# johannah/drqv2

Hardware: AMD Instinct MI355X
Metric: agent updates/sec (batch=256, 9x84x84 obs) (higher is better)
Workload: dtype f32; 1 GPU; cheetah_run batch_size=256/GPU (256 global) 9x84x84 u8 obs, A=6, feature_dim=50, hidden_dim=1024, fp32, use_tb=True; parallelism=dp1, global_batch=256

## Files before the change

drqv2_amd/_lib.py:

```python
import ctypes as C
import os

HERE = os.path.dirname(os.path.abspath(__file__))
LIB_PATH = os.path.join(HERE, "libdrqv2_hip.so")

c_float_p = C.c_void_p
c_u8_p = C.c_void_p
stream_t = C.c_void_p


class DrqStep(C.Structure):
    _fields_ = [
        ("B", C.c_int), ("global_B", C.c_int), ("C", C.c_int), ("A", C.c_int), ("F", C.c_int), ("H", C.c_int),
        ("obs", c_u8_p), ("next_obs", c_u8_p),
        ("action", c_float_p), ("reward", c_float_p), ("discount", c_float_p),
        ("shift_obs", c_float_p), ("shift_next", c_float_p),
        ("noise_critic", c_float_p), ("noise_actor", c_float_p),
        ("base_grid", c_float_p),
        ("params", c_float_p), ("grads", c_float_p), ("adam_m", c_float_p), ("adam_v", c_float_p),
        ("ws", c_float_p), ("ws_bytes", C.c_size_t),
        ("sums", c_float_p),
        ("lr", C.c_double), ("tau", C.c_double),
        ("std", C.c_float), ("clip", C.c_float),
        ("step_critic", C.c_long), ("step_enc", C.c_long), ("step_actor", C.c_long),
# ... 6 lines not shown
        ("timing_n", C.c_int),
        ("obs_index", C.c_void_p), ("next_obs_index", C.c_void_p),
        ("flags", C.c_int),
    ]


I, L, F, D, P, SZ = C.c_int, C.c_long, C.c_float, C.c_double, C.c_void_p, C.c_size_t

PROTOTYPES = {
    "drq_abi_version": (I, []),
    "drq_aug_fwd": (I, [P, P, P, P, I, I, I, I, I, P]),
    "drq_aug_fwd_f32": (I, [P, P, P, P, I, I, I, I, P]),
    "drq_conv1_aug_fwd": (I, [P, P, P, P, P, P, P, P, P, I, I, P]),
    "drq_conv1_aug_fwd_bf16": (I, [P, P, P, P, P, P, P, P, P, I, I, P]),
    "drq_conv1_aug_fwd_bf16_nhwc": (I, [P, P, P, P, P, P, P, P, P, I, I, P]),
    "drq_conv1_aug_fwd_indexed": (I, [P, P, P, P, P, P, P, P, P, P, P, I, I, P]),
    "drq_conv3x3_fwd": (I, [P, P, P, P, I, I, I, I, I, L, L, L, L, P]),
    "drq_conv3x3_dgrad": (I, [P, P, P, P, I, I, L, L, L, L, P]),
    "drq_conv3x3_fwd_wino": (I, [P, P, P, P, I, I, I, L, L, L, L, P]),
    "drq_conv3x3_dgrad_wino": (I, [P, P, P, P, I, I, L, L, L, L, P]),
    "drq_conv3x3_wgrad_wino": (I, [P, P, P, P, I, I, L, L, L, L, P, SZ, P]),
    "drq_conv3x3_wgrad": (I, [P, P, P, P, I, I, I, I, L, L, L, L, P, SZ, P]),
    "drq_conv3x3_wgrad_ws_bytes": (SZ, []),
    "drq_conv3x3_fwd_bf16": (I, [P, P, P, P, I, I, I, L, L, L, L, P]),
    "drq_conv3x3_dgrad_bf16": (I, [P, P, P, P, I, I, L, L, L, L, P]),
    "drq_conv3x3_wgrad_bf16": (I, [P, P, P, P, I, I, L, L, L, L, P, SZ, P]),
    "drq_conv3x3_fwd_bf16_nhwc": (I, [P, P, P, P, I, I, I, I, I, P]),
    "drq_conv3x3_dgrad_bf16_nhwc": (I, [P, P, P, P, I, I, I, I, L, L, L, L, P]),
    "drq_conv3x3_wgrad_bf16_nhwc": (I, [P, P, P, P, I, I, I, L, L, L, L, P, SZ, P]),
    "drq_gemm_f32": (I, [P, L, I, P, L, I, P, L, I, I, I, I, L, L, L, P, L, I, P, I, L, I, I, I, P, SZ, P]),
    "drq_gemm_batched_f32": (I, [I, P, L, I, P, L, I, P, L, I, I, I, P, I, P, I, P, I, I, I, P, SZ, P]),
    "drq_gemm_batched_bf16": (I, [I, P, L, I, P, L, I, P, L, I, I, I, P, I, P, I, P, I, I, P, SZ, P]),
    "drq_gemm_batched_partial": (I, [I, P, L, I, P, L, I, P, L, I, I, I, P, P, SZ, C.POINTER(I), P]),
    "drq_mlp_fwd": (I, [I, P, L, P, L, P, L, I, I, I, P, I, P, P, C.POINTER(I), P]),
    "drq_mlp_dgrad": (I, [I, P, L, P, L, P, L, I, I, I, P, I, P]),
    "drq_mlp_wgrad_dgrad": (I, [I, P, L, P, L, P, P, P, L, P, L, P, I, I, I, I, P]),
    "drq_ln_l1_fwd": (I, [I, P, P, P, P, P, P, P, P, P, P, P, P, P, P, P, P, P, I, I, I, L, P]),
    "drq_policy_out_l1_fwd": (I, [P, P, P, P, I, I, I, I, I, F, F, I, P, P, P, L, P, P, P, L, I, P, P, P, P]),
    "drq_qout_fwd": (I, [I, P, P, P, P, I, I, P]),
    "drq_qout_bwd": (I, [I, P, P, P, P, P, P, I, I, P]),
    "drq_ln_tanh_fwd_multi": (I, [I, P, I, P, P, P, P, P, P, I, I, P]),
    "drq_ln_tanh_fwd": (I, [P, I, P, P, P, I, P, P, I, I, P]),
    "drq_ln_tanh_fwd2": (I, [P, P, I, P, P, P, P, P, I, P, I, P, P, P, P, I, I, P]),
    "drq_ln_tanh_bwd": (I, [P, I, P, I, P, I, P, P, P, P, P, P, P, I, I, P]),
    "drq_colsum": (I, [P, L, L, P, L, I, I, I, P]),
    "drq_trunc_normal_sample": (I, [P, P, F, F, I, P, P, L, I, I, P]),
    "drq_copy_cols": (I, [P, I, P, L, I, I, P]),
    "drq_td_mse": (I, [P, P, P, P, P, P, P, P, P, I, F, P]),
    "drq_td_mse_w": (I, [P, P, P, P, P, P, P, P, P, P, P, I, F, P]),
    "drq_actor_loss": (I, [P, P, P, L, P, F, P, P, P, I, I, F, P]),
    "drq_actor_dmu": (I, [P, P, L, I, P, P, I, I, P]),
    "drq_actor_loss_bc": (I, [P, P, P, L, P, L, P, F, F, P, P, P, I, I, F, P]),
    "drq_qout_bwd_actor_bc": (I, [P, P, P, L, P, L, P, F, F, I, F, P, P, P, P, I, I, P]),
    "drq_actor_dmu_bc": (I, [P, P, L, I, P, P, L, P, L, F, P, I, I, P]),
    "drq_policy_out_bwd_bc": (I, [P, P, L, I, P, P, L, P, L, F, P, P, P, P, P, I, I, I, P, I, P]),
    "drq_adam_flat": (I, [P, P, P, P, L, D, L, F, P, D, P]),
    "drq_ema_flat": (I, [P, P, L, D, P]),
    "drq_sum_slices": (I, [P, L, I, P, L, P]),
    "drq_adam_reduce_flat": (I, [P, P, L, I, P, P, L, D, L, F, P]),
    "drq_fill": (I, [P, L, F, P]),
    "drq_u8_normalize": (I, [P, P, L, P]),
    "drq_nstep_gather": (I, [P, P, P, P, P, I, I, L, I, F, P, P, P, P, P, P]),
    "drq_tanh": (I, [P, P, L, P]),
    "drq_per_fill": (I, [P, L, L, L, I, P]),
    "drq_per_sample": (I, [P, L, P, I, I, L, D, P, P, P]),
    "drq_per_update": (I, [P, L, P, P, I, D, D, P]),
# ... 75 lines not shown
```

drqv2_amd/csrc/gemm2.hip:

```cpp
#include "common.h"
#include "internal.h"

namespace {

constexpr int MAXB2 = 8;

struct G2Args {
  const float* A[MAXB2];
  const float* B[MAXB2];
  float* C[MAXB2];
  const float* bias[MAXB2];
  const float* aux[MAXB2];
  float* rowsum[MAXB2];
  long lda, ldb, ldc;
  int ldaux;
  int M, N, K;
  int relu;
  unsigned a_bytes, b_bytes;
};

__device__ __forceinline__ int rowmap2(int r, int half) { return (r & 3) + 8 * (r >> 2) + 4 * half; }

template <bool KC>
__device__ __forceinline__ void load_step(float (&v)[16], __amdgpu_buffer_rsrc_t rs, unsigned voff, unsigned soff,
                                          unsigned ldbytes) {
  if constexpr (KC) {
#pragma unroll
    for (int q = 0; q < 4; ++q) {
      const f32x4 t = __builtin_bit_cast(
          f32x4, __builtin_amdgcn_raw_buffer_load_b128(rs, voff, soff + q * 32, 0));
      const float t0 = t[0], t1 = t[1], t2 = t[2], t3 = t[3];
      v[q * 4 + 0] = t0; v[q * 4 + 1] = t1; v[q * 4 + 2] = t2; v[q * 4 + 3] = t3;
    }
  } else {
// ... 375 lines not shown
        lsoff = (unsigned)tt * 128u + (unsigned)(st * 32) * ldb4;
        lld = ldb4;
      }
#pragma unroll
      for (int e = 0; e < 16; e += 2) {
        b[(s + D) % NS][e] = __uint_as_float(
            __builtin_amdgcn_raw_buffer_load_b32(brs, bvoff, lsoff + (8 * (e >> 2) + (e & 3)) * lld, 0));
        b[(s + D) % NS][e + 1] = __uint_as_float(
            __builtin_amdgcn_raw_buffer_load_b32(brs, bvoff, lsoff + (8 * ((e + 1) >> 2) + ((e + 1) & 3)) * lld, 0));
        __builtin_amdgcn_sched_barrier(0);
        acc0 = __builtin_amdgcn_mfma_f32_32x32x2f32(a[s][e], b[s % NS][e], acc0, 0, 0, 0);
        acc1 = __builtin_amdgcn_mfma_f32_32x32x2f32(a[s][e + 1], b[s % NS][e + 1], acc1, 0, 0, 0);
        __builtin_amdgcn_sched_barrier(0);
      }
    }
    const int n = t * 32 + col;
#pragma unroll
    for (int r = 0; r < 16; ++r) {
      const int row = mt * 32 + rowmap2(r, half);
      if (row < g.M) c[(long)row * g.ldc + n] = acc0[r] + acc1[r];
    }
  }
  if (g.rowsum && grp == 0) {
    float rs = 0.f;
#pragma unroll
    for (int s = 0; s < KSTEPS; ++s)
#pragma unroll
      for (int e = 0; e < 16; ++e) rs += a[s][e];
    rs += __shfl_xor(rs, 32);
    if (half == 0 && m < g.M) g.rowsum[m] = rs;
  }
}

}

int drq_trunk_wgrad_ln(const float* A, long lda, const float* B, long ldb, float* C, long ldc, int M, int N, int K,
                       float* rowsum, const float* ln_dln, const float* ln_xhat, float* ln_dgamma, float* ln_dbeta,
                       int ln_rows, int ln_F, hipStream_t st) {
  if (M < 1 || M > 128 || N < 4096 || N % 32 || (K != 128 && K != 256 && K != 512)) return DRQ_EARG;
  if (ln_rows > 0 && (!ln_dln || !ln_xhat || !ln_dgamma || !ln_dbeta || ln_F < 1 || ln_F > 256)) return DRQ_EARG;
  const size_t ab = (size_t)K * lda * 4, bb = (size_t)K * ldb * 4;
  if (ab >= (1ull << 31) || bb >= (1ull << 31)) return DRQ_EARG;
  TWArgs g{A, B, C, rowsum, lda, ldb, ldc, M, N, K, (unsigned)ab, (unsigned)bb,
           ln_dln, ln_xhat, ln_dgamma, ln_dbeta, ln_rows > 0 ? ln_rows : 0, ln_F};
  const int blocks = drq_num_cus() + (ln_rows > 0 ? 1 : 0);
  if (K == 512) hipLaunchKernelGGL((trunk_wgrad_kernel<16>), dim3(blocks), dim3(256), 0, st, g);
  else if (K == 256) hipLaunchKernelGGL((trunk_wgrad_kernel<8>), dim3(blocks), dim3(256), 0, st, g);
  else hipLaunchKernelGGL((trunk_wgrad_kernel<4>), dim3(blocks), dim3(256), 0, st, g);
  DRQ_LAUNCH_CHECK();
  return DRQ_OK;
}

int drq_trunk_wgrad(const float* A, long lda, const float* B, long ldb, float* C, long ldc, int M, int N, int K,
                    float* rowsum, hipStream_t st) {
  return drq_trunk_wgrad_ln(A, lda, B, ldb, C, ldc, M, N, K, rowsum, nullptr, nullptr, nullptr, nullptr, 0, 0, st);
}

int drq_trunk_fwd_partial(int nbatch, const float* const* A, long lda, const float* const* B, long ldb, int M, int N,
                          int K, float* ws, size_t ws_bytes, int* splitk_out, hipStream_t st) {
  if (nbatch <= 0 || nbatch > MAXB2 || M % 32 || M < 32 || N < 1 || N > 128 || K % 32 || K < 4096) return DRQ_EARG;
  if (lda % 4 || ldb % 4 || !ws || ((uintptr_t)ws & 15)) return DRQ_EARG;
  const size_t ab = (size_t)M * lda * 4, bb = (size_t)N * ldb * 4;
  if (ab >= (1ull << 31) || bb >= (1ull << 31)) return DRQ_EARG;
  TrunkArgs g{};
  for (int b = 0; b < nbatch; ++b) {
    if (((uintptr_t)A[b] & 15) || ((uintptr_t)B[b] & 15)) return DRQ_EARG;
    g.A[b] = A[b]; g.B[b] = B[b];
  }
  g.part = ws; g.lda = lda; g.ldb = ldb; g.M = M; g.N = N; g.K = K;
  g.a_bytes = (unsigned)ab; g.b_bytes = (unsigned)bb;
  const int steps = K / 32, cus = drq_num_cus();
  const bool wide = N > 64;
// ... 38 lines not shown
  if (a_kc && !b_kc) return launch2<true, false>(g, nbatch, st);
  return launch2<false, false>(g, nbatch, st);
}

int drq_gemm2_wgrad_dgrad(int nbatch, const float* const* dy, long lddy, const float* const* x, long ldx,
                          float* const* dw, float* const* db, const float* const* w, long ldw, float* const* dx,
                          long lddx, const float* const* mask, int ldmask, int Brows, int Nout, int Kin, hipStream_t st) {
  if (nbatch <= 0 || nbatch > MAXB2 || Brows % 32 || Nout % 32 || Kin % 32 || Brows < 64 || Nout < 64 || Kin < 32)
    return DRQ_EARG;
  if (lddy % 4) return DRQ_EARG;
  G2Args gw{}, gd{};
  for (int b = 0; b < nbatch; ++b) {
    if (!dy[b] || !x[b] || !dw[b] || !w[b] || !dx[b] || ((uintptr_t)dy[b] & 15)) return DRQ_EARG;
    gw.A[b] = dy[b]; gw.B[b] = x[b]; gw.C[b] = dw[b]; gw.rowsum[b] = db ? db[b] : nullptr;
    gd.A[b] = dy[b]; gd.B[b] = w[b]; gd.C[b] = dx[b]; gd.aux[b] = mask ? mask[b] : nullptr;
  }
  gw.lda = lddy; gw.ldb = ldx; gw.ldc = Kin; gw.M = Nout; gw.N = Kin; gw.K = Brows;
  gd.lda = lddy; gd.ldb = ldw; gd.ldc = lddx; gd.ldaux = ldmask; gd.M = Brows; gd.N = Kin; gd.K = Nout;
  const size_t dyb = (size_t)Brows * lddy * 4, xb = (size_t)Brows * ldx * 4, wb = (size_t)Nout * ldw * 4;
  if (dyb >= (1ull << 31) || xb >= (1ull << 31) || wb >= (1ull << 31)) return DRQ_EARG;
  gw.a_bytes = (unsigned)dyb; gw.b_bytes = (unsigned)xb;
  gd.a_bytes = (unsigned)dyb; gd.b_bytes = (unsigned)wb;
  const bool sw = gemm2_split(gw, nbatch), sd = gemm2_split(gd, nbatch);
  const int tw = (gw.M / 32) * (gw.N / 32), td = (gd.M / 32) * (gd.N / 32);
  const int nxw = sw ? tw : (tw + 3) / 4, nxd = sd ? td : (td + 3) / 4;
  const dim3 grid(nxw + nxd, 1, nbatch);
  if (sw && sd) hipLaunchKernelGGL((gemm2_pair_kernel<4, 4>), grid, dim3(256), 0, st, gw, gd, nxw);
  else if (sw) hipLaunchKernelGGL((gemm2_pair_kernel<4, 1>), grid, dim3(256), 0, st, gw, gd, nxw);
  else if (sd) hipLaunchKernelGGL((gemm2_pair_kernel<1, 4>), grid, dim3(256), 0, st, gw, gd, nxw);
  else hipLaunchKernelGGL((gemm2_pair_kernel<1, 1>), grid, dim3(256), 0, st, gw, gd, nxw);
  DRQ_LAUNCH_CHECK();
  return DRQ_OK;
}
```

drqv2_amd/csrc/internal.h:

```cpp
#pragma once
#include "common.h"

int drq_ln_tanh_fwd_multi_ex(int n, const float* const* z, int ldz, const float* const* gamma,
                             const float* const* beta, float* const* out, const int* ldo, float* const* xhat,
                             float* const* rstd, int rows, int F, const float* const* tail, const int* tail_ld,
                             int tail_n, hipStream_t st);
int drq_ln_tanh_fwd_multi_part(int n, const float* const* z, int ldz, const float* const* gamma,
                               const float* const* beta, float* const* out, const int* ldo, float* const* xhat,
                               float* const* rstd, int rows, int F, const float* const* tail, const int* tail_ld,
                               int tail_n, const float* part, const float* const* bias, int splitk, hipStream_t st);
int drq_ln_tanh_bwd_part(const float* dh0, int ld0, const float* dh1, int ld1, const float* h, int ldh,
                         const float* xhat, const float* rstd, const float* gamma, float* dz, float* dln,
                         float* dgamma, float* dbeta, int rows, int F, const float* part, int splitk, int nprob,
                         int ldp, hipStream_t st);
int drq_ln_param_grad(const float* dln, const float* xhat, float* dgamma, float* dbeta, int rows, int F,
                      hipStream_t st);
int drq_qout_bwd_td(const float* tq1, const float* tq2, const float* q1, const float* q2, const float* reward,
                    const float* discount, float inv_global_B, float* sums, const float* const* h,
                    const float* const* w, float* const* dh, float* const* dw, float* const* db, int B, int H,
                    hipStream_t st);
int drq_qout_bwd_td_w(const float* tq1, const float* tq2, const float* q1, const float* q2, const float* reward,
                      const float* discount, const float* is_weight, float inv_global_B, float* sums, float* td_abs,
                      const float* const* h, const float* const* w, float* const* dh, float* const* dw,
                      float* const* db, int B, int H, hipStream_t st);
// ... 6 lines not shown
                       hipStream_t st);
int drq_policy_out_bwd(const float* da1, const float* da2, long ld, int col0, const float* mu, const float* p2,
                       const float* w, float* dp2, float* dw, float* db, int B, int H, int A, const float* part,
                       int splitk, hipStream_t st);
int drq_actor_loss_ex(const float* q1, const float* q2, const float* a, long lda, const float* mu, float std,
                      float* dq1, float* dq2, float* sums, int B, int A, float inv_global_B, float* sums_host,
                      unsigned seq, hipStream_t st);
int drq_actor_loss_bc_ex(const float* q1, const float* q2, const float* a, long lda, const float* a_beh, long ldb,
                         const float* mu, float std, float alpha, float* dq1, float* dq2, float* sums, int B, int A,
                         float inv_global_B, float* sums_host, unsigned seq, hipStream_t st);
int drq_qout_bwd_actor_bc_ex(const float* q1, const float* q2, const float* act, long lda, const float* a_beh, long ldb,
                             const float* mu, float std, float alpha, int A, float inv_global_B, float* sums,
                             float* sums_host, unsigned seq, const float* const* h, const float* const* w,
                             float* const* dh, int B, int H, hipStream_t st);
int drq_adam_flat2(float* p0, const float* g0, float* m0, float* v0, long n0, long step0, float* p1, const float* g1,
                   float* m1, float* v1, long n1, long step1, double lr, float gscale, hipStream_t st);

int drq_gemm_batched_any(int bf16, int nbatch, const float* const* A, long lda, int a_kc, const float* const* B, long ldb,
                         int b_kc, float* const* C, long ldc, int M, int N, int K, const float* const* bias, int relu,
                         const float* const* aux, int ldaux, float* const* rowsum, int scatter_hw, int tile,
                         int splitk, float* ws, size_t ws_bytes, hipStream_t st);
int drq_gemm_batched_partial_any(int bf16, int nbatch, const float* const* A, long lda, int a_kc, const float* const* B,
                                 long ldb, int b_kc, float* const* C, long ldc, int M, int N, int K,
                                 const float* const* bias, float* ws, size_t ws_bytes, int* splitk_out, hipStream_t st);

int drq_skinny_dgrad(const float* dz, long lda, const float* w, long ldb, float* c, long ldc, int M, int N, int K,
                     const float* aux, int ldaux, int scatter_hw, hipStream_t st);

int drq_trunk_wgrad(const float* A, long lda, const float* B, long ldb, float* C, long ldc, int M, int N, int K,
                    float* rowsum, hipStream_t st);
int drq_trunk_wgrad_ln(const float* A, long lda, const float* B, long ldb, float* C, long ldc, int M, int N, int K,
                       float* rowsum, const float* ln_dln, const float* ln_xhat, float* ln_dgamma, float* ln_dbeta,
                       int ln_rows, int ln_F, hipStream_t st);
int drq_trunk_fwd_partial(int nbatch, const float* const* A, long lda, const float* const* B, long ldb, int M, int N,
                          int K, float* ws, size_t ws_bytes, int* splitk_out, hipStream_t st);
int drq_gemm2(int nbatch, const float* const* A, long lda, int a_kc, const float* const* B, long ldb, int b_kc,
              float* const* C, long ldc, int M, int N, int K, const float* const* bias, int relu,
              const float* const* aux, int ldaux, float* const* rowsum, hipStream_t st);
int drq_gemm2_wgrad_dgrad(int nbatch, const float* const* dy, long lddy, const float* const* x, long ldx,
                          float* const* dw, float* const* db, const float* const* w, long ldw, float* const* dx,
                          long lddx, const float* const* mask, int ldmask, int Brows, int Nout, int Kin, hipStream_t st);

int drq_gemm3_dgrad(int nbatch, const float* const* dy, long lddy, const float* const* w, long ldw, float* const* dx,
                    long lddx, int M, int N, int K, const float* const* mask, int ldmask, hipStream_t st);
int drq_gemm3_wgrad_dgrad(int nbatch, const float* const* dy, long lddy, const float* const* x, long ldx,
                          float* const* dw, float* const* db, const float* const* w, long ldw, float* const* dx,
                          long lddx, const float* const* mask, int ldmask, int Brows, int Nout, int Kin, hipStream_t st);

int drq_lnl1_fwd(int njobs, const float* const* part, const float* const* z, const float* const* bias,
                 const float* const* gamma, const float* const* beta, float* const* out, const int* ldo,
                 float* const* xhat, float* const* rstd, const float* const* tail, const int* tail_ld, const int* tail_n,
                 const int* rows, const int* nheads, const float* const* w, const float* const* b, float* const* y, int F,
                 int H, int splitk, long slab, hipStream_t st);
int drq_polout_l1_fwd(const float* p2, const float* w3, const float* b3, float* p3, int rows, int srow0, int H, int A,
                      int F, float std, float clip, int use_clip, const float* noise_hi, float* mu_hi, float* ha_hi,
                      long lda_hi, const float* noise_lo, float* mu_lo, float* ha_lo, long lda_lo, int nheads,
                      const float* const* w, const float* const* b, float* const* y, hipStream_t st);

int drq_conv1_aug_fwd_any(int bf_mma, const uint8_t* obs, const float* shift, const uint8_t* obs1, const float* shift1,
                          const float* base_grid, const float* w, const float* bias, float* xaug, float* y, int n,
                          int n_store, hipStream_t st, const float* const* wino_w, float* wino_u, const long* fidx0,
                          const long* fidx1);

int drq_conv3x3_fwd_wino_pre(const float* x, const float* w, const float* u_image, const float* bias, float* y, int nb,
                             int hin, int relu, long y_bs, long y_cs, long y_rs, long y_off, hipStream_t st);
int drq_conv3x3_dgrad_wino_pre(const float* dy_pad, const float* w, const float* u_image, const float* mask, float* dx,
// ... 35 lines not shown
```

drqv2_amd/csrc/step.hip:

```cpp
#include "common.h"
#include "internal.h"
#include "../../include/drqv2_hip.h"

namespace {

constexpr long R = 32L * 35 * 35;
inline long al64(long x) { return (x + 63) & ~63L; }
inline long al512(long x) { return (x + 511) & ~511L; }

struct HeadOff {
  long trunk_w, trunk_b, ln_g, ln_b;
  long w[2][3], b[2][3];
};
enum { SEG_ENC, SEG_CRITIC, SEG_ACTOR, SEG_TARGET };
struct ParamLayout {
  long enc_w[4], enc_b[4];
  HeadOff critic, actor, target;
  long seg[8];
  long total;
  long flat[50];
  int nflat;
  long seg_beg(int net) const { return seg[2 * net]; }
  long seg_len(int net) const { return seg[2 * net + 1] - seg[2 * net]; }
};
// ... 124 lines not shown
  take(W_GEMM_WS, kGemmWsFloats);
  take(W_CONV_WS, (long)(drq_conv3x3_wgrad_ws_bytes() / sizeof(float)));
  take(W_WINO_U, 6L * 16384);
  w.total = off;
  return w;
}

#define CK(expr)                \
  do {                          \
    const int rc__ = (expr);    \
    if (rc__ != 0) return rc__; \
  } while (0)

struct Ctx {
  const DrqStep* s;
  ParamLayout P;
  WsLayout W;
  hipStream_t st;
  bool fuse_actor_loss = false;
  float bc_alpha = 0.f;
  bool bc() const { return bc_alpha > 0.f; }
  const float* a_beh() const { return ws(W_HA_C) + s->F; }
  float bc_scale() const { return 2.0f / ((float)s->global_B * (float)s->A); }
  const float* is_weight = nullptr;
  float* td_abs = nullptr;
  bool per() const { return is_weight != nullptr; }
  bool qout_loss_fits_lds() const { return ((size_t)s->B + 5 * 1024 + 16) * 4 <= 60 * 1024; }
  bool actor_loss_fused() const { return fuse_actor_loss && qout_loss_fits_lds(); }
  bool fuse_rows() const {
    return !(s->flags & DRQ_STEP_NO_ROW_FUSION) && !s->bf16 && s->A <= 32 && s->F + s->A <= 64 && s->F % 2 == 0 &&
           s->A % 2 == 0 && s->H % 256 == 0;
  }
  bool use_gemm3() const { return !(s->flags & DRQ_STEP_NO_GEMM3) && !s->bf16; }
  int stamp(int idx) const {
    if (s->timing_events && idx < s->timing_n && hipEventRecord((hipEvent_t)s->timing_events[idx], st) != hipSuccess)
      return DRQ_EARG;
    return 0;
  }
  float* ws(int id) const { return s->ws + W.off[id]; }
  float* p(long off) const { return s->params + off; }
  float* g(long off) const { return s->grads + off; }
  int bf16() const { return s->bf16 ? 1 : 0; }
  bool acts16() const { return s->bf16 && !(s->flags & DRQ_STEP_BF16_FP32_ACTS); }
  bool grads16() const { return acts16() && !(s->flags & DRQ_STEP_BF16_FP32_GRADS); }
  int adam_segment(int net, long step, int target = -1) const {
    const long o = P.seg_beg(net);
    return drq_adam_flat(p(o), g(o), s->adam_m + o, s->adam_v + o, P.seg_len(net), s->lr, step, s->gscale,
                         target >= 0 ? p(P.seg_beg(target)) : nullptr, target >= 0 ? s->tau : 0.0, st);
  }
  float* gemm_ws() const { return ws(W_GEMM_WS); }
  size_t gemm_ws_bytes() const { return (size_t)kGemmWsFloats * sizeof(float); }

  int fwd(int n, const float* const* x, long ldx, const float* const* w, const float* const* b, float* const* y,
          long ldy, int M, int N, int K, int relu) const {
    return drq_gemm_batched_any(bf16(), n, x, ldx, 1, w, K, 1, y, ldy, M, N, K, b, relu, nullptr, 0, nullptr, 0, 0, 0,
                                gemm_ws(), gemm_ws_bytes(), st);
  }
  int dgrad(int n, const float* const* dy, long lddy, const float* const* w, long ldw, float* const* dx, long lddx,
            int M, int Nout, int K, const float* const* mask, int ldmask) const {
    if (use_gemm3() && n >= 2 && K >= 256 && Nout >= 256) {
      const int rc = drq_gemm3_dgrad(n, dy, lddy, w, ldw, dx, lddx, M, Nout, K, mask, ldmask, st);
      if (rc != DRQ_EARG) return rc;
    }
    return drq_gemm_batched_any(bf16(), n, dy, lddy, 1, w, ldw, 0, dx, lddx, M, Nout, K, nullptr, 0, mask, ldmask, nullptr, 0,
                                0, 0, gemm_ws(), gemm_ws_bytes(), st);
  }
// ... 218 lines not shown
    const float *w0[2] = {c.p(cr.w[0][0]), c.p(cr.w[1][0])}, *w1[2] = {c.p(cr.w[0][1]), c.p(cr.w[1][1])},
                *w2[2] = {c.p(cr.w[0][2]), c.p(cr.w[1][2])};
    float *gw0[2] = {c.g(cr.w[0][0]), c.g(cr.w[1][0])}, *gw1[2] = {c.g(cr.w[0][1]), c.g(cr.w[1][1])},
          *gw2[2] = {c.g(cr.w[0][2]), c.g(cr.w[1][2])};
    float *gb0[2] = {c.g(cr.b[0][0]), c.g(cr.b[1][0])}, *gb1[2] = {c.g(cr.b[0][1]), c.g(cr.b[1][1])},
          *gb2[2] = {c.g(cr.b[0][2]), c.g(cr.b[1][2])};
    if (c.qout_loss_fits_lds() && c.per()) {
      CK(drq_qout_bwd_td_w(c.ws(W_TQ), c.ws(W_TQ) + B, c.ws(W_Q), c.ws(W_Q) + B, s->reward, s->discount, c.is_weight,
                           invB, s->sums, c.td_abs, c2c, w2, dc2, gw2, gb2, B, H, st));
    } else if (c.qout_loss_fits_lds()) {
      CK(drq_qout_bwd_td(c.ws(W_TQ), c.ws(W_TQ) + B, c.ws(W_Q), c.ws(W_Q) + B, s->reward, s->discount, invB, s->sums,
                         c2c, w2, dc2, gw2, gb2, B, H, st));
    } else {
      if (c.per())
        CK(drq_td_mse_w(c.ws(W_TQ), c.ws(W_TQ) + B, c.ws(W_Q), c.ws(W_Q) + B, s->reward, s->discount, c.is_weight,
                        c.ws(W_DQ), c.ws(W_DQ) + B, c.td_abs, s->sums, B, invB, st));
      else
        CK(drq_td_mse(c.ws(W_TQ), c.ws(W_TQ) + B, c.ws(W_Q), c.ws(W_Q) + B, s->reward, s->discount, c.ws(W_DQ),
                      c.ws(W_DQ) + B, s->sums, B, invB, st));
      CK(drq_qout_bwd(2, dq, c2c, w2, dc2, gw2, gb2, B, H, st));
    }
    CK(c.wgrad_dgrad(2, dc2c, H, c1c, H, gw1, gb1, w1, H, dc1, H, c1c, H, B, H, H));
    CK(c.wgrad(2, dc1c, H, hac, FA, gw0, gb0, B, H, FA));
    CK(drq_gemm_batched_partial_any(c.bf16(), 2, dc1c, H, 1, w0, FA, 0, dha, FA, B, FA, H, nullptr, c.gemm_ws(), c.gemm_ws_bytes(),
                                &sk_dha, st));
  }
  const bool ride = c.ln_rides();
  CK(drq_ln_tanh_bwd_part(c.ws(W_DHA), FA, c.ws(W_DHA) + (long)B * FA, FA, c.ws(W_HA_C), FA, c.ws(W_XHAT_C),
                          c.ws(W_RSTD_C), c.p(cr.ln_g), c.ws(W_DZ_C), c.ws(W_DLN), ride ? nullptr : c.g(cr.ln_g),
                          ride ? nullptr : c.g(cr.ln_b), B, F, sk_dha > 1 ? c.gemm_ws() : nullptr, sk_dha, 2, FA, st));
  {
    const float *dz[1] = {c.ws(W_DZ_C)}, *w[1] = {c.p(cr.trunk_w)}, *mk[1] = {feat_obs};
    float* dy4[1] = {c.ws(W_DY4)};
    CK(c.trunk_wgrad(c.ws(W_DZ_C), feat_obs, c.g(cr.trunk_w), c.g(cr.trunk_b), ride, c.ws(W_DLN), c.ws(W_XHAT_C),
                     c.g(cr.ln_g), c.g(cr.ln_b)));
    CK(drq_gemm_batched_any(0, 1, dz, F, 1, w, R, 0, dy4, 0, B, (int)R, F, nullptr, 0, mk, (int)R, nullptr, 35, 0, 0,
                            c.gemm_ws(), c.gemm_ws_bytes(), st));
  }

  return 0;
}

int phase_conv_backward(const Ctx& c) {
  const DrqStep* s = c.s;
  const ParamLayout& P = c.P;
  const int B = s->B, C = s->C;
  hipStream_t st = c.st;
  const int dyid[4] = {W_DY1, W_DY2, W_DY3, W_DY4};
  const int actid[4] = {W_AUG, W_ACT1, W_ACT2, W_ACT3};
  float* cws = c.ws(W_CONV_WS);
  const size_t quarter = drq_conv3x3_wgrad_ws_bytes() / 4;
  const float* parts[4];
  int nblk[4], cins[4];
  float *dws[4], *dbs[4];
  const bool merged = !c.bf16();
  for (int l = 3; l >= 0; --l) {
    const int hin = kEncH[l], hout = kEncH[l + 1], hp = hout + 4;
    const float* dy = c.ws(dyid[l]);
    float* part = cws + (size_t)l * (quarter / sizeof(float));
    parts[l] = part; cins[l] = l == 0 ? C : 32; dws[l] = c.g(P.enc_w[l]); dbs[l] = c.g(P.enc_b[l]);
    if (!merged) {
      if (l > 0)
        CK(drq_conv3x3_wgrad_partial_bf16_lay(c.ws(actid[l]), dy, B, hin, 32L * hp * hp, (long)hp * hp, hp, 2L * hp + 2,
                                              part, quarter, &nblk[l],
                                              (c.acts16() ? 1 : 0) | (c.grads16() && l < 3 ? 2 : 0), st));
      else
        CK(drq_conv3x3_wgrad_partial(c.ws(actid[l]), dy, B, C, hin, 2, 32L * hp * hp, (long)hp * hp, hp, 2L * hp + 2,
                                     part, quarter, &nblk[l], st));
    }
    if (l >= 1) {
// ... 343 lines not shown
```

drqv2_amd/ops.py:

```python
import torch

from . import _lib
from ._lib import check, ptr

ENC_H = (84, 41, 39, 37, 35)


def _alloc(shape, dtype, device, kind="out"):
    if kind == "zero":
        return torch.zeros(shape, device=device, dtype=dtype)
    return torch.empty(shape, device=device, dtype=dtype)


def _stream():
    return torch.cuda.current_stream().cuda_stream


def _need(t, dtype=torch.float32, name="tensor"):
    if not (isinstance(t, torch.Tensor) and t.is_cuda):
        raise _lib.DrqError(f"{name}: a GPU tensor is required (the HIP path has no CPU fallback)")
    if t.device.index != torch.cuda.current_device():
        raise _lib.DrqError(f"{name} lives on {t.device} but the current device is cuda:{torch.cuda.current_device()}: "
                            "wrap the call in torch.cuda.device(...)")
    if t.dtype != dtype or not t.is_contiguous():
# ... 214 lines not shown
    c_bs = c_bs if c_bs is not None else M * N
    if out is None:
        out = _alloc((nbatch, M, N) if nbatch > 1 else (M, N), torch.float32, dev)
    if ws is None:
        ws = _alloc((16 * 1024 * 1024,), torch.float32, dev, "ws")
    check(lib.drq_gemm_f32(ptr(A), lda, int(a_kc), ptr(B), ldb, int(b_kc), ptr(out), ldc, M, N, K, nbatch, a_bs, b_bs,
                           c_bs, ptr(bias), bias_bs, int(relu), ptr(aux), (aux.shape[-1] if aux is not None else 0),
                           aux_bs, 0, tile, splitk, ptr(ws), ws.numel() * 4, _stream()), "drq_gemm_f32")
    return out


def linear_fwd(x, w, b, relu=False, **kw):
    M, K = x.shape
    N = w.shape[0]
    return gemm(x, True, w, True, M, N, K, bias=b, relu=relu, **kw)


def linear_dgrad(dy, w, mask=None, **kw):
    M, K = dy.shape
    N = w.shape[1]
    return gemm(dy, True, w, False, M, N, K, aux=mask, **kw)


def linear_wgrad(dy, x, **kw):
    Brows, N = dy.shape
    K = x.shape[1]
    dw = gemm(dy, False, x, False, N, K, Brows, lda=N, ldb=K, **kw)
    lib = _lib.load()
    db = _alloc((N,), torch.float32, dy.device)
    check(lib.drq_colsum(ptr(dy), N, 0, ptr(db), 0, Brows, N, 1, _stream()), "drq_colsum")
    return dw, db


def ln_tanh_fwd(z, gamma, beta, save=True):
    lib = _lib.load()
    rows, F = z.shape
    out = _alloc(z.shape, z.dtype, z.device)
    xhat = _alloc(z.shape, z.dtype, z.device) if save else None
    rstd = _alloc((rows,), torch.float32, z.device) if save else None
    check(lib.drq_ln_tanh_fwd(ptr(z), F, ptr(gamma), ptr(beta), ptr(out), F, ptr(xhat), ptr(rstd), rows, F, _stream()),
          "drq_ln_tanh_fwd")
    return out, xhat, rstd


def ln_tanh_bwd(dh, h, xhat, rstd, gamma):
    lib = _lib.load()
    rows, F = dh.shape
    dz, dln = _alloc(dh.shape, dh.dtype, dh.device), _alloc(dh.shape, dh.dtype, dh.device)
    dg, db = _alloc(gamma.shape, gamma.dtype, gamma.device), _alloc(gamma.shape, gamma.dtype, gamma.device)
    check(lib.drq_ln_tanh_bwd(ptr(dh), F, None, 0, ptr(h), F, ptr(xhat), ptr(rstd), ptr(gamma), ptr(dz), ptr(dln),
                              ptr(dg), ptr(db), rows, F, _stream()), "drq_ln_tanh_bwd")
    return dz, dg, db


def trunc_normal_sample(pre_tanh, noise, std, clip):
    lib = _lib.load()
    B, A = pre_tanh.shape
    mu, a = (_alloc(pre_tanh.shape, pre_tanh.dtype, pre_tanh.device) for _ in range(2))
    check(lib.drq_trunc_normal_sample(ptr(pre_tanh), ptr(noise), float(std), float(clip if clip is not None else 0.0),
                                      int(clip is not None), ptr(mu), ptr(a), A, B, A, _stream()),
          "drq_trunc_normal_sample")
    return mu, a


def adam_flat(p, g, m, v, lr, step, gscale=1.0, tgt=None, tau=0.0):
    lib = _lib.load()
# ... 222 lines not shown
```

include/drqv2_hip.h:

```cpp
#ifndef DRQV2_HIP_H
#define DRQV2_HIP_H
#include <stddef.h>
#include <stdint.h>

#ifdef __cplusplus
extern "C" {
#endif

typedef void* drq_stream_t;

#define DRQ_OK 0
#define DRQ_EARG (-1)
#define DRQ_EWS (-2)

int drq_abi_version(void);

int drq_aug_fwd(const uint8_t* obs, const float* shift_xy, const float* base_grid, float* out, int n, int c,
                int hw, int pad, int fuse_norm, drq_stream_t stream);
int drq_aug_fwd_f32(const float* x, const float* shift_xy, const float* base_grid, float* out, int n, int c,
                    int hw, int pad, drq_stream_t stream);

int drq_conv1_aug_fwd(const uint8_t* obs, const float* shift, const uint8_t* obs1, const float* shift1,
                      const float* base_grid, const float* w, const float* bias, float* xaug, float* y, int n,
                      int n_store, drq_stream_t stream);
// ... 25 lines not shown
int drq_conv3x3_fwd_bf16(const float* x, const float* w, const float* bias, float* y, int nb, int hin, int relu,
                         long y_bs, long y_cs, long y_rs, long y_off, drq_stream_t stream);
int drq_conv3x3_dgrad_bf16(const float* dy_pad, const float* w, const float* mask, float* dx, int nb, int hout,
                           long dx_bs, long dx_cs, long dx_rs, long dx_off, drq_stream_t stream);
int drq_conv3x3_wgrad_bf16(const float* x, const float* dy, float* dw, float* db, int nb, int hin, long dy_bs,
                           long dy_cs, long dy_rs, long dy_off, float* ws, size_t ws_bytes, drq_stream_t stream);
int drq_conv3x3_fwd_bf16_nhwc(const void* x, const float* w, const float* bias, void* y, int nb, int hin, int relu,
                              int x_nhwc, int y_nhwc, drq_stream_t stream);
int drq_conv3x3_dgrad_bf16_nhwc(const void* dy_pad, const float* w, const void* mask_nhwc, void* dx, int nb, int hout,
                                int dy_nhwc, int dx_nhwc, long dx_bs, long dx_cs, long dx_rs, long dx_off,
                                drq_stream_t stream);
int drq_conv3x3_wgrad_bf16_nhwc(const void* x_nhwc, const void* dy, float* dw, float* db, int nb, int hin, int dy_nhwc,
                                long dy_bs, long dy_cs, long dy_rs, long dy_off, float* ws, size_t ws_bytes,
                                drq_stream_t stream);

int drq_gemm_f32(const float* A, long lda, int a_kc, const float* B, long ldb, int b_kc, float* C, long ldc,
                 int M, int N, int K, int nbatch, long a_bs, long b_bs, long c_bs, const float* bias, long bias_bs,
                 int relu, const float* aux, int ldaux, long aux_bs, int scatter_hw, int tile, int splitk,
                 float* ws, size_t ws_bytes, drq_stream_t stream);

int drq_gemm_batched_f32(int nbatch, const float* const* A, long lda, int a_kc, const float* const* B, long ldb,
                         int b_kc, float* const* C, long ldc, int M, int N, int K, const float* const* bias, int relu,
                         const float* const* aux, int ldaux, float* const* rowsum, int scatter_hw, int tile,
                         int splitk, float* ws, size_t ws_bytes, drq_stream_t stream);

int drq_gemm_batched_bf16(int nbatch, const float* const* A, long lda, int a_kc, const float* const* B, long ldb,
                          int b_kc, float* const* C, long ldc, int M, int N, int K, const float* const* bias, int relu,
                          const float* const* aux, int ldaux, float* const* rowsum, int scatter_hw, int splitk,
                          float* ws, size_t ws_bytes, drq_stream_t stream);

int drq_gemm_batched_partial(int nbatch, const float* const* A, long lda, int a_kc, const float* const* B, long ldb,
                             int b_kc, float* const* C, long ldc, int M, int N, int K, const float* const* bias,
                             float* ws, size_t ws_bytes, int* splitk_out, drq_stream_t stream);

int drq_mlp_fwd(int nbatch, const float* const* x, long ldx, const float* const* w, long ldw, float* const* y,
                long ldy, int M, int N, int K, const float* const* bias, int relu, const float* const* qw,
                float* const* qpart, int* nq_out, drq_stream_t stream);
int drq_mlp_dgrad(int nbatch, const float* const* dy, long lddy, const float* const* w, long ldw, float* const* dx,
                  long lddx, int M, int N, int K, const float* const* mask, int ldmask, drq_stream_t stream);
int drq_mlp_wgrad_dgrad(int nbatch, const float* const* dy, long lddy, const float* const* x, long ldx,
                        float* const* dw, float* const* db, const float* const* w, long ldw, float* const* dx,
                        long lddx, const float* const* mask, int ldmask, int Brows, int Nout, int Kin,
                        drq_stream_t stream);

int drq_ln_l1_fwd(int njobs, const float* const* part, const float* const* z, const float* const* bias,
                  const float* const* gamma, const float* const* beta, float* const* out, const int* ldo,
                  float* const* xhat, float* const* rstd, const float* const* tail, const int* tail_ld,
                  const int* tail_n, const int* rows, const int* nheads, const float* const* w, const float* const* b,
                  float* const* y, int F, int H, int splitk, long slab, drq_stream_t stream);
int drq_policy_out_l1_fwd(const float* p2, const float* w3, const float* b3, float* p3, int rows, int srow0, int H, int A,
                          int F, float std, float clip, int use_clip, const float* noise_hi, float* mu_hi, float* ha_hi,
                          long lda_hi, const float* noise_lo, float* mu_lo, float* ha_lo, long lda_lo, int nheads,
                          const float* const* w, const float* const* b, float* const* y, drq_stream_t stream);

int drq_qout_fwd(int nz, const float* const* h, const float* const* w, const float* const* b, float* const* q, int B,
                 int H, drq_stream_t stream);
int drq_qout_bwd(int nz, const float* const* dq, const float* const* h, const float* const* w, float* const* dh,
                 float* const* dw, float* const* db, int B, int H, drq_stream_t stream);

int drq_ln_tanh_fwd(const float* z, int ldz, const float* gamma, const float* beta, float* out, int ldo,
                    float* xhat, float* rstd, int rows, int F, drq_stream_t stream);
int drq_ln_tanh_fwd2(const float* z0, const float* z1, int ldz, const float* gamma0, const float* beta0,
                     const float* gamma1, const float* beta1, float* out0, int ldo0, float* out1, int ldo1,
                     float* xhat0, float* rstd0, float* xhat1, float* rstd1, int rows, int F, drq_stream_t stream);
int drq_ln_tanh_fwd_multi(int n, const float* const* z, int ldz, const float* const* gamma, const float* const* beta,
                          float* const* out, const int* ldo, float* const* xhat, float* const* rstd, int rows, int F,
// ... 71 lines not shown
  const float* action;
  const float* reward;
  const float* discount;
  const float* shift_obs;
  const float* shift_next;
  const float* noise_critic;
  const float* noise_actor;
  const float* base_grid;
  float* params;
  float* grads;
  float* adam_m;
  float* adam_v;
  float* ws;
  size_t ws_bytes;
  float* sums;
  double lr, tau;
  float std, clip;
  long step_critic, step_enc, step_actor;
  float gscale;
  drq_stream_t stream;
  float* sums_host;
  int store_aug_next;
  int bf16;
  void* const* timing_events;
  int timing_n;
  const int64_t* obs_index;
  const int64_t* next_obs_index;
  int flags;
} DrqStep;
#define DRQ_STEP_NO_ROW_FUSION 1
#define DRQ_STEP_NO_GEMM3 2
#define DRQ_STEP_BF16_FP32_ACTS 4
#define DRQ_STEP_BF16_FP32_GRADS 8

int drq_param_layout(int C, int A, int F, int H, long* out, int cap);
#define DRQ_PARAM_LAYOUT_LEN 59

size_t drq_step_ws_bytes(int B, int C, int A, int F, int H);
long drq_step_ws_offset(int B, int C, int A, int F, int H, int buffer_id);
enum {
  DRQ_WS_AUG = 0, DRQ_WS_ACT1, DRQ_WS_ACT2, DRQ_WS_ACT3, DRQ_WS_FEAT, DRQ_WS_Z_NEXT, DRQ_WS_Z_OBS,
  DRQ_WS_HA_T, DRQ_WS_HA_C, DRQ_WS_H_AN, DRQ_WS_H_AO, DRQ_WS_Q, DRQ_WS_TQ, DRQ_WS_DQ, DRQ_WS_MU_O,
  DRQ_WS_DY4, DRQ_WS_DY3, DRQ_WS_DY2, DRQ_WS_DY1, DRQ_WS_DZ_C, DRQ_WS_DZ_A, DRQ_WS_HA_C2,
  DRQ_WS_P1, DRQ_WS_P2,
  DRQ_WS_C1, DRQ_WS_C2,
  DRQ_WS_NBUF_PUBLIC
};

enum {
  DRQ_PHASE_ALL = -1, DRQ_PHASE_CRITIC = 0, DRQ_PHASE_ACTOR = 1, DRQ_PHASE_OPT = 2,
  DRQ_PHASE_ENCODE = 3, DRQ_PHASE_CRITIC_HEADS = 4, DRQ_PHASE_CONV_BACKWARD = 5, DRQ_PHASE_ACTOR_FORWARD = 6,
  DRQ_PHASE_ACTOR_BACKWARD = 7, DRQ_PHASE_ENCODER_OPT = 8, DRQ_PHASE_ACTOR_OPT = 9,
  DRQ_PHASE_CRITIC_OPT = 10, DRQ_PHASE_ACTOR_LOSS = 11, DRQ_PHASE_POLYAK = 12, DRQ_PHASE_REDRAW = 13
};
int drq_update_phase(const DrqStep* s, int phase);
int drq_update_phase_bc(const DrqStep* s, int phase, float bc_alpha);
int drq_update_phase_per(const DrqStep* s, int phase, const float* is_weight, float* td_abs);

int drq_publish_sums(const float* sums, float* sums_host, unsigned seq, drq_stream_t stream);

int drq_act_forward(const DrqStep* s, const uint8_t* obs, int n, float* mu_out);

size_t drq_act_ws_bytes(int n_max, int C, int A, int F, int H);
int drq_act_batch(const float* params, int C, int A, int F, int H, const uint8_t* obs, int n, const float* noise,
                  float std, float* mu_out, float* action_out, void* ws, size_t ws_bytes, drq_stream_t stream);

// ... 5 lines not shown
```

Baseline: 978.5 updates/s.

## Fuse critic trunk weight-gradient and input-gradient into one MFMA kernel

Adds a single kernel that computes the trunk weight gradient (dz^T·feat) and the ReLU-masked, scatter-padded input gradient (dz·W) in the same pass over column tiles. It reuses the feature tile loaded for the wgrad as the ReLU mask and stages dz^T in LDS. It replaces the separate trunk_wgrad launch and skinny dgrad GEMM in the critic conv-backward phase. The goal is to save one launch and a second read of feat and W. The cost is a complex hand-scheduled kernel with large register and LDS use at one block per CU. It falls back to the old path on argument errors and can be turned off with a new flag.

```diff
diff --git a/drqv2_amd/_lib.py b/drqv2_amd/_lib.py
--- a/drqv2_amd/_lib.py
+++ b/drqv2_amd/_lib.py
@@ -62,6 +62,7 @@
     "drq_gemm_batched_f32": (I, [I, P, L, I, P, L, I, P, L, I, I, I, P, I, P, I, P, I, I, I, P, SZ, P]),
     "drq_gemm_batched_bf16": (I, [I, P, L, I, P, L, I, P, L, I, I, I, P, I, P, I, P, I, I, P, SZ, P]),
     "drq_gemm_batched_partial": (I, [I, P, L, I, P, L, I, P, L, I, I, I, P, P, SZ, C.POINTER(I), P]),
+    "drq_trunk_bwd_fused": (I, [P, P, P, P, P, P, I, I, I, I, P, P, P, P, I, P]),
     "drq_mlp_fwd": (I, [I, P, L, P, L, P, L, I, I, I, P, I, P, P, C.POINTER(I), P]),
     "drq_mlp_dgrad": (I, [I, P, L, P, L, P, L, I, I, I, P, I, P]),
     "drq_mlp_wgrad_dgrad": (I, [I, P, L, P, L, P, P, P, L, P, L, P, I, I, I, I, P]),
diff --git a/drqv2_amd/csrc/gemm2.hip b/drqv2_amd/csrc/gemm2.hip
--- a/drqv2_amd/csrc/gemm2.hip
+++ b/drqv2_amd/csrc/gemm2.hip
@@ -1,5 +1,7 @@
 #include "common.h"
 #include "internal.h"
+#include "../../include/drqv2_hip.h"
+#include <type_traits>
 
 namespace {
 
@@ -441,12 +443,235 @@
   }
 }
 
+struct TBArgs {
+  TWArgs w;
+  const float* wt;
+  float* dx;
+  long ldw, crow;
+  int scatter_hw;
+  unsigned w_bytes, dx_bytes;
+};
+
+template <int KSTEPS, int KP, int MT>
+__global__ __launch_bounds__(256, 1) void trunk_bwd_kernel(TBArgs ga) {
+  constexpr int NS = 4, D = 3;
+  constexpr int MP = KSTEPS * 32 + 33;
+  constexpr int NPAIR = KSTEPS * 8;
+  static_assert(KSTEPS % NS == 0, "stage index must be a compile-time constant");
+  static_assert(KSTEPS % MT == 0 && (MT == 2 || MT == 4), "every wave of a group takes the same number of steps");
+  extern __shared__ float dzt[];
+  const TWArgs& g = ga.w;
+  const int nblk = (int)gridDim.x - (g.ln_rows > 0 ? 1 : 0);
+  if (g.ln_rows > 0 && (int)blockIdx.x == nblk) {
+    ln_param_rider(g);
+    return;
+  }
+  const int tid = threadIdx.x, lane = tid & 63;
+  const int wid = __builtin_amdgcn_readfirstlane(threadIdx.x >> 6);
+  const int col = lane & 31, half = lane >> 5;
+  const int ntiles = g.N >> 5;
+  const int gw = (int)blockIdx.x * 4 + wid, nw = nblk * 4;
+  const int mt = gw % MT, grp = gw / MT, ngrp = nw / MT;
+  const int per = ntiles / ngrp, rem = ntiles - per * ngrp;
+  const int t0 = grp * per + (grp < rem ? grp : rem);
+  const int t1 = t0 + per + (grp < rem ? 1 : 0);
+  const bool live = t0 < t1;
+
+  const __amdgpu_buffer_rsrc_t ars = __builtin_amdgcn_make_buffer_rsrc((void*)g.A, 0, g.a_bytes, 0x00020000);
+  const __amdgpu_buffer_rsrc_t brs = __builtin_amdgcn_make_buffer_rsrc((void*)g.B, 0, g.b_bytes, 0x00020000);
+  const __amdgpu_buffer_rsrc_t wrs = __builtin_amdgcn_make_buffer_rsrc((void*)ga.wt, 0, ga.w_bytes, 0x00020000);
+  const __amdgpu_buffer_rsrc_t xrs = __builtin_amdgcn_make_buffer_rsrc((void*)ga.dx, 0, ga.dx_bytes, 0x00020000);
+  const unsigned lda4 = (unsigned)g.lda * 4, ldb4 = (unsigned)g.ldb * 4, ldw4 = (unsigned)ga.ldw * 4;
+  const unsigned crow4 = (unsigned)ga.crow * 4;
+  const int m = mt * 32 + col;
+  const unsigned avoff = m < g.M ? (unsigned)(half * 4) * lda4 + (unsigned)m * 4 : 0x7ffffff0u;
+  const unsigned bvoff = (unsigned)(half * 4) * ldb4 + (unsigned)col * 4;
+  const unsigned wvoff = (unsigned)half * ldw4 + (unsigned)col * 4;
+
+  float a[KSTEPS][16];
+  float b[NS][16];
+  float wv[KP], wvn[KP];
+  const int total = (t1 - t0) * KSTEPS;
+  if (live) {
+#pragma unroll
+    for (int s = 0; s < KSTEPS; ++s) load_step<false>(a[s], ars, avoff, (unsigned)(s * 32) * lda4, lda4);
+#pragma unroll
+    for (int i = 0; i < D; ++i) {
+      const int ic = i < total ? i : total - 1;
+      const int t = t0 + ic / KSTEPS, st = ic % KSTEPS;
+      load_step<false>(b[i], brs, bvoff, (unsigned)t * 128u + (unsigned)(st * 32) * ldb4, ldb4);
+    }
+#pragma unroll
+    for (int kp = 0; kp < KP; ++kp)
+      wv[kp] = __uint_as_float(
+          __builtin_amdgcn_raw_buffer_load_b32(wrs, wvoff, (unsigned)t0 * 128u + (unsigned)(2 * kp) * ldw4, 0));
+  }
+  for (int idx = tid; idx < KSTEPS * 32 * 2 * KP; idx += 256) {
+    const int r = idx / (2 * KP), k = idx - r * (2 * KP);
+    dzt[k * MP + r] = g.A[(long)r * g.lda + k];
+  }
+  __syncthreads();
+  if (!live) return;
+
+  const float* ap0 = dzt + half * MP + col;
+  float* c = g.C;
+  auto run = [&](auto mti_c) {
+  constexpr int MTI = decltype(mti_c)::value;
+  for (int t = t0; t < t1; ++t) {
+    f32x16 acc0, acc1;
+#pragma unroll
+    for (int r = 0; r < 16; ++r) { acc0[r] = 0.f; acc1[r] = 0.f; }
+    const int ibase = (t - t0) * KSTEPS;
+    const int n = t * 32 + col;
+    long cn = n;
+    if (ga.scatter_hw > 0) {
+      const int hw = ga.scatter_hw, hp = hw + 4;
+      const int ch = n / (hw * hw);
+      const int rr = n - ch * hw * hw;
+      const int y = rr / hw, x = rr - y * hw;
+      cn = ((long)ch * hp + (y + 2)) * hp + (x + 2);
+    }
+    const unsigned xvoff = (unsigned)cn * 4 + (unsigned)(4 * half) * crow4;
+    const unsigned wsoff = (unsigned)(t + 1 < t1 ? t + 1 : t) * 128u;
+#pragma unroll
+    for (int s = 0; s < KSTEPS; ++s) {
+      unsigned lsoff;
+      {
+        const int i = ibase + s + D, ic = i < total ? i : total - 1;
+        const int tt = t0 + ic / KSTEPS, st = ic % KSTEPS;
+        lsoff = (unsigned)tt * 128u + (unsigned)(st * 32) * ldb4;
+      }
+      auto pair = [&](int e) {
+        b[(s + D) % NS][e] = __uint_as_float(
+            __builtin_amdgcn_raw_buffer_load_b32(brs, bvoff, lsoff + (8 * (e >> 2) + (e & 3)) * ldb4, 0));
+        b[(s + D) % NS][e + 1] = __uint_as_float(
+            __builtin_amdgcn_raw_buffer_load_b32(brs, bvoff, lsoff + (8 * ((e + 1) >> 2) + ((e + 1) & 3)) * ldb4, 0));
+#pragma unroll
+        for (int kp = 0; kp < KP; ++kp)
+          if ((kp * (NPAIR / 2)) / KP == s * 8 + (e >> 1))
+            wvn[kp] = __uint_as_float(
+                __builtin_amdgcn_raw_buffer_load_b32(wrs, wvoff, wsoff + (unsigned)(2 * kp) * ldw4, 0));
+        __builtin_amdgcn_sched_barrier(0);
+        acc0 = __builtin_amdgcn_mfma_f32_32x32x2f32(a[s][e], b[s % NS][e], acc0, 0, 0, 0);
+        acc1 = __builtin_amdgcn_mfma_f32_32x32x2f32(a[s][e + 1], b[s % NS][e + 1], acc1, 0, 0, 0);
+      };
+      if ((s % MT) == (MTI >= 0 ? MTI : mt)) {
+        constexpr int AVH = KP > 32 ? (KP + 1) / 2 : KP;
+        float av[AVH];
+        const float* ap = ap0 + s * 32;
+        const unsigned xv = xvoff + (unsigned)(s * 32) * crow4;
+#pragma unroll
+        for (int kp = 0; kp < AVH; ++kp) av[kp] = ap[2 * kp * MP];
+        pair(0);
+        __builtin_amdgcn_sched_barrier(0);
+        f32x16 accd;
+#pragma unroll
+        for (int r = 0; r < 16; ++r) accd[r] = 0.f;
+#pragma unroll
+        for (int kp = 0; kp < AVH; ++kp) accd = __builtin_amdgcn_mfma_f32_32x32x2f32(av[kp], wv[kp], accd, 0, 0, 0);
+        if constexpr (KP > AVH) {
+          __builtin_amdgcn_sched_barrier(0);
+#pragma unroll
+          for (int kp = AVH; kp < KP; ++kp) av[kp - AVH] = ap[2 * kp * MP];
+#pragma unroll
+          for (int kp = AVH; kp < KP; ++kp)
+            accd = __builtin_amdgcn_mfma_f32_32x32x2f32(av[kp - AVH], wv[kp], accd, 0, 0, 0);
+        }
+        __builtin_amdgcn_sched_barrier(0);
+#pragma unroll
+        for (int e = 2; e < 16; e += 2) {
+          pair(e);
+#pragma unroll
+          for (int r = 0; r < 16; ++r)
+            if ((r * 7) / 16 + 1 == (e >> 1)) {
+              const float v = b[s % NS][r] > 0.f ? accd[r] : 0.f;
+              __builtin_amdgcn_raw_buffer_store_b32(__float_as_uint(v), xrs, xv,
+                                                    (unsigned)((r & 3) + 8 * (r >> 2)) * crow4, 0);
+            }
+          __builtin_amdgcn_sched_barrier(0);
+        }
+      } else {
+#pragma unroll
+        for (int e = 0; e < 16; e += 2) {
+          pair(e);
+          __builtin_amdgcn_sched_barrier(0);
+        }
+      }
+    }
+#pragma unroll
+    for (int r = 0; r < 16; ++r) {
+      const int row = mt * 32 + rowmap2(r, half);
+      if (row < g.M) c[(long)row * g.ldc + n] = acc0[r] + acc1[r];
+    }
+#pragma unroll
+    for (int kp = 0; kp < KP; ++kp) wv[kp] = wvn[kp];
+  }
+  };
+  if constexpr (MT == 2) {
+    if (mt == 0) run(std::integral_constant<int, 0>{});
+    else run(std::integral_constant<int, 1>{});
+  } else {
+    run(std::integral_constant<int, -1>{});
+  }
+  if (g.rowsum && grp == 0) {
+    float rs = 0.f;
+#pragma unroll
+    for (int s = 0; s < KSTEPS; ++s)
+#pragma unroll
+      for (int e = 0; e < 16; ++e) rs += a[s][e];
+    rs += __shfl_xor(rs, 32);
+    if (half == 0 && m < g.M) g.rowsum[m] = rs;
+  }
+}
+
+template <int KSTEPS, int KP, int MT>
+int launch_trunk_bwd(const TBArgs& g, int blocks, hipStream_t st) {
+  constexpr int lds = 2 * KP * (KSTEPS * 32 + 33) * 4;
+  static_assert(lds + 2 * 4 * 64 * 4 <= 160 * 1024, "dz^T image + the rider's scratch must fit the LDS");
+  static bool attr_dev[kMaxDevices] = {};
+  bool& attr = attr_dev[drq_device()];
+  if (!attr) {
+    const hipError_t e = hipFuncSetAttribute((const void*)trunk_bwd_kernel<KSTEPS, KP, MT>,
+                                             hipFuncAttributeMaxDynamicSharedMemorySize, lds);
+    if (e != hipSuccess) return (int)e;
+    attr = true;
+  }
+  hipLaunchKernelGGL((trunk_bwd_kernel<KSTEPS, KP, MT>), dim3(blocks), dim3(256), lds, st, g);
+  DRQ_LAUNCH_CHECK();
+  return DRQ_OK;
+}
+
+}
+
+int drq_trunk_bwd(const float* dz, long lddz, const float* feat, long ldf, const float* w, long ldw, float* dw,
+                  long lddw, float* db, float* dx, long lddx, int scatter_hw, int M, int N, int K,
+                  const float* ln_dln, const float* ln_xhat, float* ln_dgamma, float* ln_dbeta, int ln_rows, int ln_F,
+                  hipStream_t st) {
+  if (!dz || !feat || !w || !dw || !dx) return DRQ_EARG;
+  if ((M != 50 && M != 100) || N < 32 || N % 32 || (K != 128 && K != 256 && K != 512)) return DRQ_EARG;
+  if (K == 512) return DRQ_EARG;
+  if (ln_rows > 0 && (!ln_dln || !ln_xhat || !ln_dgamma || !ln_dbeta || ln_F < 1 || ln_F > 256)) return DRQ_EARG;
+  if (scatter_hw > 0 && N != 32 * scatter_hw * scatter_hw) return DRQ_EARG;
+  const long crow = scatter_hw > 0 ? 32L * (scatter_hw + 4) * (scatter_hw + 4) : lddx;
+  if (lddz < M || ldf < N || ldw < N || lddw < N || crow < N) return DRQ_EARG;
+  const size_t ab = (size_t)K * lddz * 4, bb = (size_t)K * ldf * 4, wb = (size_t)M * ldw * 4, xb = (size_t)K * crow * 4;
+  if (ab >= (1ull << 31) || bb >= (1ull << 31) || wb >= (1ull << 31) || xb >= (1ull << 31)) return DRQ_EARG;
+  TBArgs g{{dz, feat, dw, db, lddz, ldf, lddw, M, N, K, (unsigned)ab, (unsigned)bb,
+            ln_dln, ln_xhat, ln_dgamma, ln_dbeta, ln_rows > 0 ? ln_rows : 0, ln_F},
+           w, dx, ldw, crow, scatter_hw, (unsigned)wb, (unsigned)xb};
+  const int blocks = drq_num_cus() + (ln_rows > 0 ? 1 : 0);
+  if (M == 50) {
+    if (K == 256) return launch_trunk_bwd<8, 25, 2>(g, blocks, st);
+    return launch_trunk_bwd<4, 25, 2>(g, blocks, st);
+  }
+  if (K == 256) return launch_trunk_bwd<8, 50, 4>(g, blocks, st);
+  return launch_trunk_bwd<4, 50, 4>(g, blocks, st);
 }
 
 int drq_trunk_wgrad_ln(const float* A, long lda, const float* B, long ldb, float* C, long ldc, int M, int N, int K,
                        float* rowsum, const float* ln_dln, const float* ln_xhat, float* ln_dgamma, float* ln_dbeta,
                        int ln_rows, int ln_F, hipStream_t st) {
-  if (M < 1 || M > 128 || N < 4096 || N % 32 || (K != 128 && K != 256 && K != 512)) return DRQ_EARG;
+  if (M < 1 || M > 128 || N < 32 || N % 32 || (K != 128 && K != 256 && K != 512)) return DRQ_EARG;
   if (ln_rows > 0 && (!ln_dln || !ln_xhat || !ln_dgamma || !ln_dbeta || ln_F < 1 || ln_F > 256)) return DRQ_EARG;
   const size_t ab = (size_t)K * lda * 4, bb = (size_t)K * ldb * 4;
   if (ab >= (1ull << 31) || bb >= (1ull << 31)) return DRQ_EARG;
@@ -551,3 +776,18 @@
   DRQ_LAUNCH_CHECK();
   return DRQ_OK;
 }
+
+DRQ_API int drq_trunk_bwd_fused(const float* dz, const float* feat, const float* w, float* dw, float* db, float* dfeat,
+                                int B, int F, int N, int scatter_hw, const float* ln_dln, const float* ln_xhat,
+                                float* ln_dgamma, float* ln_dbeta, int fused, drq_stream_t stream) {
+  if (!dz || !feat || !w || !dw || !db || !dfeat || B <= 0 || F <= 0 || N <= 0) return DRQ_EARG;
+  if (scatter_hw > 0 && N != 32 * scatter_hw * scatter_hw) return DRQ_EARG;
+  hipStream_t st = (hipStream_t)stream;
+  const int ln_rows = ln_dln ? B : 0;
+  if (fused)
+    return drq_trunk_bwd(dz, F, feat, N, w, N, dw, N, db, dfeat, N, scatter_hw, F, N, B, ln_dln, ln_xhat, ln_dgamma,
+                         ln_dbeta, ln_rows, F, st);
+  const int rc = drq_trunk_wgrad_ln(dz, F, feat, N, dw, N, F, N, B, db, ln_dln, ln_xhat, ln_dgamma, ln_dbeta, ln_rows, F, st);
+  if (rc != DRQ_OK) return rc;
+  return drq_skinny_dgrad(dz, F, w, N, dfeat, N, B, N, F, feat, N, scatter_hw, st);
+}
diff --git a/drqv2_amd/csrc/internal.h b/drqv2_amd/csrc/internal.h
--- a/drqv2_amd/csrc/internal.h
+++ b/drqv2_amd/csrc/internal.h
@@ -62,6 +62,10 @@
 int drq_trunk_wgrad_ln(const float* A, long lda, const float* B, long ldb, float* C, long ldc, int M, int N, int K,
                        float* rowsum, const float* ln_dln, const float* ln_xhat, float* ln_dgamma, float* ln_dbeta,
                        int ln_rows, int ln_F, hipStream_t st);
+int drq_trunk_bwd(const float* dz, long lddz, const float* feat, long ldf, const float* w, long ldw, float* dw,
+                  long lddw, float* db, float* dx, long lddx, int scatter_hw, int M, int N, int K,
+                  const float* ln_dln, const float* ln_xhat, float* ln_dgamma, float* ln_dbeta, int ln_rows, int ln_F,
+                  hipStream_t st);
 int drq_trunk_fwd_partial(int nbatch, const float* const* A, long lda, const float* const* B, long ldb, int M, int N,
                           int K, float* ws, size_t ws_bytes, int* splitk_out, hipStream_t st);
 int drq_gemm2(int nbatch, const float* const* A, long lda, int a_kc, const float* const* B, long ldb, int b_kc,
diff --git a/drqv2_amd/csrc/step.hip b/drqv2_amd/csrc/step.hip
--- a/drqv2_amd/csrc/step.hip
+++ b/drqv2_amd/csrc/step.hip
@@ -180,6 +180,7 @@
            s->A % 2 == 0 && s->H % 256 == 0;
   }
   bool use_gemm3() const { return !(s->flags & DRQ_STEP_NO_GEMM3) && !s->bf16; }
+  bool fuse_trunk_bwd() const { return !(s->flags & DRQ_STEP_NO_TRUNK_BWD_FUSION) && !s->bf16; }
   int stamp(int idx) const {
     if (s->timing_events && idx < s->timing_n && hipEventRecord((hipEvent_t)s->timing_events[idx], st) != hipSuccess)
       return DRQ_EARG;
@@ -464,10 +465,20 @@
   {
     const float *dz[1] = {c.ws(W_DZ_C)}, *w[1] = {c.p(cr.trunk_w)}, *mk[1] = {feat_obs};
     float* dy4[1] = {c.ws(W_DY4)};
-    CK(c.trunk_wgrad(c.ws(W_DZ_C), feat_obs, c.g(cr.trunk_w), c.g(cr.trunk_b), ride, c.ws(W_DLN), c.ws(W_XHAT_C),
-                     c.g(cr.ln_g), c.g(cr.ln_b)));
-    CK(drq_gemm_batched_any(0, 1, dz, F, 1, w, R, 0, dy4, 0, B, (int)R, F, nullptr, 0, mk, (int)R, nullptr, 35, 0, 0,
-                            c.gemm_ws(), c.gemm_ws_bytes(), st));
+    bool fused = false;
+    if (ride && c.fuse_trunk_bwd()) {
+      const int rc = drq_trunk_bwd(c.ws(W_DZ_C), F, feat_obs, R, c.p(cr.trunk_w), R, c.g(cr.trunk_w), R, c.g(cr.trunk_b),
+                                   c.ws(W_DY4), 0, 35, F, (int)R, B, c.ws(W_DLN), c.ws(W_XHAT_C), c.g(cr.ln_g),
+                                   c.g(cr.ln_b), B, F, st);
+      if (rc == DRQ_OK) fused = true;
+      else if (rc != DRQ_EARG) return rc;
+    }
+    if (!fused) {
+      CK(c.trunk_wgrad(c.ws(W_DZ_C), feat_obs, c.g(cr.trunk_w), c.g(cr.trunk_b), ride, c.ws(W_DLN), c.ws(W_XHAT_C),
+                       c.g(cr.ln_g), c.g(cr.ln_b)));
+      CK(drq_gemm_batched_any(0, 1, dz, F, 1, w, R, 0, dy4, 0, B, (int)R, F, nullptr, 0, mk, (int)R, nullptr, 35, 0, 0,
+                              c.gemm_ws(), c.gemm_ws_bytes(), st));
+    }
   }
 
   return 0;
diff --git a/drqv2_amd/ops.py b/drqv2_amd/ops.py
--- a/drqv2_amd/ops.py
+++ b/drqv2_amd/ops.py
@@ -270,6 +270,23 @@
     return dw, db
 
 
+def trunk_bwd(dz, feat, w, fused=True, scatter_hw=0, ln=None, dfeat=None):
+    lib = _lib.load()
+    B, F = dz.shape
+    N = feat.shape[1]
+    dev = dz.device
+    dw = _alloc((F, N), torch.float32, dev)
+    db = _alloc((F,), torch.float32, dev)
+    if dfeat is None:
+        dfeat = _alloc((B, N), torch.float32, dev)
+    dln, xhat = ln if ln is not None else (None, None)
+    dg = _alloc((F,), torch.float32, dev) if ln is not None else None
+    dbt = _alloc((F,), torch.float32, dev) if ln is not None else None
+    check(lib.drq_trunk_bwd_fused(ptr(dz), ptr(feat), ptr(w), ptr(dw), ptr(db), ptr(dfeat), B, F, N, scatter_hw, ptr(dln),
+                                  ptr(xhat), ptr(dg), ptr(dbt), int(fused), _stream()), "drq_trunk_bwd_fused")
+    return dw, db, dfeat, ((dg, dbt) if ln is not None else None)
+
+
 def ln_tanh_fwd(z, gamma, beta, save=True):
     lib = _lib.load()
     rows, F = z.shape
diff --git a/include/drqv2_hip.h b/include/drqv2_hip.h
--- a/include/drqv2_hip.h
+++ b/include/drqv2_hip.h
@@ -81,6 +81,10 @@
 int drq_gemm_batched_partial(int nbatch, const float* const* A, long lda, int a_kc, const float* const* B, long ldb,
                              int b_kc, float* const* C, long ldc, int M, int N, int K, const float* const* bias,
                              float* ws, size_t ws_bytes, int* splitk_out, drq_stream_t stream);
+
+int drq_trunk_bwd_fused(const float* dz, const float* feat, const float* w, float* dw, float* db, float* dfeat,
+                        int B, int F, int N, int scatter_hw, const float* ln_dln, const float* ln_xhat,
+                        float* ln_dgamma, float* ln_dbeta, int fused, drq_stream_t stream);
 
 int drq_mlp_fwd(int nbatch, const float* const* x, long ldx, const float* const* w, long ldw, float* const* y,
                 long ldy, int M, int N, int K, const float* const* bias, int relu, const float* const* qw,
@@ -218,6 +222,7 @@
 #define DRQ_STEP_NO_GEMM3 2
 #define DRQ_STEP_BF16_FP32_ACTS 4
 #define DRQ_STEP_BF16_FP32_GRADS 8
+#define DRQ_STEP_NO_TRUNK_BWD_FUSION 16
 
 int drq_param_layout(int C, int A, int F, int H, long* out, int cap);
 #define DRQ_PARAM_LAYOUT_LEN 59
```

Measured after the change: 985.4 updates/s (median of 6 runs). No clear change (+0.7%).
